# chenxy99/Scanpaths

Hardware: AMD Instinct MI355X
Metric: images/sec/GPU (AiR train step, bs=32, 320x512) at 1/2/4/8 MI355X (higher is better)
Workload: dtype f32; 1 GPU; AiR supervised train step (fwd+loss+bwd+clip+Adam), resnet50, T=16, 320x512, per-GPU batch 32; global_batch=32, parallelism=dp1

## Files before the change

### include/scanpaths_amd.h

```cpp
#ifndef SCANPATHS_AMD_H
#define SCANPATHS_AMD_H
#include <stdint.h>

#ifdef __cplusplus
extern "C" {
#endif

#define SP_OK 0
#define SP_EINVAL (-1)
#define SP_ENULL (-2)

#define SP_ABI_VERSION 4
int sp_abi_version(void);

int sp_set_tuning(const char* name, int value);
int sp_timing_build(void);

typedef struct sp_conv_desc {
    int N_img, Hi, Wi, Kc, ldx;
    int Ho, Wo, Nout, ldc;
    int KH, KW, stride, pad, dil;
    int mode, ldw;
    float alpha;
    int beta, relu;
// ... 125 lines not shown
int sp_sempool_fwd(const float* a, const float* vf, int S, int B, int P, int C, float alpha, void* workspace, float* out, int sbc,
                   void* stream);
int sp_sempool_bwd(const float* dout, const float* out, const float* a, const float* vf, int S, int B, int P, int C, float alpha,
                   float* da, float* dvf, const int* row_last, int row_step, int sbc, void* stream);
int sp_lstm_pointwise_bwd(const float* dh, const float* dc, const float* gates, const float* c_prev, const float* c_out,
                          int64_t rows, int C, float* dpre, float* dc_prev, unsigned* dpre_amax, unsigned* dcp_amax,
                          const unsigned* dh_amax, const unsigned* dc_amax, float c_bound, float cprev_bound, void* planes,
                          float* dpre_scale, const int* row_last, int row_step, int rows_per_sample, void* stream);

int sp_im2col3x3_1ch(const float* maps, int S, int R, int H, int W, int ldk, float* col, void* stream);
int sp_col2im3x3_1ch(const float* dcol, int S, int R, int H, int W, int ldk, float* dmaps, void* stream);

int sp_listatt_fwd(const float* L, const float* u, int T, int R, int D, float* mem, float* alpha, void* stream);
int sp_listatt_bwd(const float* dmem, const float* L, const float* u, const float* alpha, int T, int R, int D, float* dL,
                   float* du_partial, void* stream);

int sp_mulrelu_fwd(const float* a, const float* b, int64_t n, int64_t nb, float* out, void* stream);
int sp_mulrelu_bwd(const float* dout, const float* a, const float* b, const float* out, int64_t n, int64_t nb, float* da,
                   float* db_partial, void* stream);

int sp_select_rows(const float* a, const float* b, const unsigned char* sel, int64_t rows, int64_t len, float* out,
                   void* stream);
int sp_select_rows_bwd(const float* dout, const unsigned char* sel, int64_t rows, int64_t len, float* da, float* db,
                       void* stream);

int sp_head_finish_fwd(const float* Z, int B, int Hm, int Wm, int ldz, int nheads, int HC, const float* cb,
                       int cb_per_sample , const float* w2, const float* b2, int softmax, float* logits, float* amap, float* mu,
                       float* sigma2, float* drt,
                       const float* dpre ,
                       int zc , int parts, void* stream);
int sp_head_finish_bwd(const float* dlogits, int64_t dlogits_ld, const float* damap , const float* dmu,
                       const float* dsigma2, const float* logits, const float* amap, const float* sigma2, const float* drt, int B, int Hm,
                       int Wm, int ldz, int nheads, int HC, const float* w2, int softmax, float* dZ, float* dcb_partial,
                       float* dw2_partial, float* db2_partial,
                       float* ddpre ,
                       int zc, int parts, int* live, void* stream);

int sp_head_num_classes(int Hm, int Wm);
int sp_head_compose11_fwd(const float* G, const float* cb, int nheads, int HC, int C, int Hm, int Wm, float* W11,
                          float* cbsum, void* stream);
int sp_head_compose11_bwd(const float* dW11, const float* dcbsum, int nheads, int HC, int C, int Hm, int Wm, float* dG,
                          float* dcb, void* stream);
int sp_sal_gather_fwd(const float* T, int B, int Hm, int Wm, int ldt, int nsel, const int* hmap, float* Z2, void* stream);
int sp_sal_gather_bwd(const float* dZ2, int B, int Hm, int Wm, int ldt, int nsel, int nsrc, const int* hmap, float* dT,
                      const int* row_last, int row_step, void* stream);
int sp_drt_direct_fwd(const float* h, const float* W11, const float* cbsum, const int* hmap, int B, int Hm, int Wm, int C,
                      int nsel, float* Dpre, void* stream);
int sp_drt_direct_bwd_data(const float* dDpre, const float* W11, const int* hmap, int B, int Hm, int Wm, int C, int nsel,
                           int accumulate, float* dh, const int* live, const int* row_last, int row_step, int rowB, void* stream);
int64_t sp_drt_direct_bwd_weight_workspace(int B, int Hm, int Wm, int C, int nsel);
int sp_drt_direct_bwd_weight(const float* dDpre, const float* h, const int* hmap, int B, int Hm, int Wm, int C, int nsel, int nheads,
                             void* workspace, float* dW11, float* dcbsum, const int* live, const int* row_last, int row_step, int rowB,
                             void* stream);

int sp_gemm_skinny_applies(int M, int N, int K, int lda, int ldb, int ldc, int layout);
int64_t sp_gemm_skinny_workspace(int M, int N, int K, int layout);
int sp_gemm_skinny(const float* A, const float* B, const float* bias, float* C, int M, int N, int K, int lda, int ldb, int ldc, int layout,
                   float alpha, int relu, void* workspace, void* stream);

int64_t sp_scanpath_loss_workspace(int B, int T);
// ... 106 lines not shown
```

### scanpaths_amd/config.py

```python
from __future__ import annotations

import os
import sys

DEFAULTS = {
    "split_scheme": "f16x2", "use_split": True, "library": "product", "always_reset_amax": False,
    "fused_amax": True, "grad_merge": True, "bn_split": True, "bn_skip_dx": True, "bn_skip_z": True, "lstm_bwd_split": True,
    "rank1_dsp_split": True, "rank1_dwc_split": True, "lstm_skip_dpre": True, "fuse_gate_lstm": True, "lstm_h_planes": True,
    "defer_wgrad": True, "channel_scales": True, "hw2_single": True, "row_sparsity": True, "direct_grad": True, "skinny_gemm": True, "async_dgrad": True,
    "drt_batched": True, "rank1_fused": True,
}
_off = lambda v: v != "0"
_ENV = {
    "SP_SPLIT_SCHEME": ("split_scheme", str), "SP_NO_SPLIT": ("use_split", lambda v: not v), "SP_LIBRARY": ("library", str),
    "SP_ALWAYS_RESET_AMAX": ("always_reset_amax", bool), "SP_NO_AMAX_HINT": ("fused_amax", lambda v: not v),
    "SP_GRAD_MERGE": ("grad_merge", _off), "SP_BN_SPLIT": ("bn_split", _off), "SP_BN_SKIP_DX": ("bn_skip_dx", _off),
    "SP_BN_SKIP_Z": ("bn_skip_z", _off), "SP_LSTM_BWD_SPLIT": ("lstm_bwd_split", _off), "SP_RANK1_DSP_SPLIT": ("rank1_dsp_split", _off),
    "SP_RANK1_DWC_SPLIT": ("rank1_dwc_split", _off), "SP_LSTM_SKIP_DPRE": ("lstm_skip_dpre", _off), "SP_FUSE_LSTM": ("fuse_gate_lstm", _off),
    "SP_LSTM_H_PLANES": ("lstm_h_planes", _off), "SP_DEFER_WGRAD": ("defer_wgrad", _off), "SP_CHANNEL_SCALES": ("channel_scales", _off),
    "SP_HW2_SINGLE": ("hw2_single", _off), "SP_ROW_SPARSITY": ("row_sparsity", _off), "SP_DIRECT_GRAD": ("direct_grad", _off), "SP_SKINNY_GEMM": ("skinny_gemm", _off),
    "SP_ASYNC_DGRAD": ("async_dgrad", _off), "SP_DRT_BATCHED": ("drt_batched", _off), "SP_RANK1_FUSED": ("rank1_fused", _off),
}
TIMING_KNOBS = {"SP_H2_DBG": b"h2_dbg", "SP_HW_DBG": b"hw_dbg", "SP_B3_DBG": b"b3_dbg", "SP_HW_SPLITS": b"hw_splits", "SP_H2_HALO": b"h2_halo",
                "SP_ROW_ORDER": b"row_order", "SP_HW_CAP": b"hw_cap"}

settings = dict(DEFAULTS)
_announced = set()


def env_tuning_allowed() -> bool:
    return os.environ.get("SP_ALLOW_ENV_TUNING") == "1"


def _loud(msg: str) -> None:
    if msg not in _announced:
        _announced.add(msg)
# ... 65 lines not shown
```

### scanpaths_amd/csrc/decoder.hip

```cpp
#include "common.h"
#include <algorithm>

namespace {

inline int ew_blocks(int64_t n) { return (int)std::max<int64_t>(1, std::min<int64_t>(sp_cdiv(n, 256), 2048)); }

__device__ __forceinline__ float sigmoidf_(float x) { return sp_sigmoid(x); }

__global__ __launch_bounds__(256) void lstm_fwd_kernel(const float* xg, const float* hg, const float* c_prev,
                                                       int64_t rows, int C, float* gates, float* c_out, float* h_out) {
    const int C4 = C / 4;
    const int64_t total = rows * C4;
    for (int64_t idx = (int64_t)blockIdx.x * blockDim.x + threadIdx.x; idx < total; idx += (int64_t)gridDim.x * blockDim.x) {
        const int64_t r = idx / C4;
        const int c = (int)(idx - r * C4) * 4;
        const float* px = xg + r * 4 * C + c;
        float4 pi = *reinterpret_cast<const float4*>(px);
        float4 pf = *reinterpret_cast<const float4*>(px + C);
        float4 po = *reinterpret_cast<const float4*>(px + 2 * C);
        float4 pg = *reinterpret_cast<const float4*>(px + 3 * C);
        if (hg) {
            const float* ph = hg + r * 4 * C + c;
            const float4 a = *reinterpret_cast<const float4*>(ph), b = *reinterpret_cast<const float4*>(ph + C);
            const float4 d = *reinterpret_cast<const float4*>(ph + 2 * C), e = *reinterpret_cast<const float4*>(ph + 3 * C);
// ... 371 lines not shown
        const int r = (int)(q % R);
        const int s = (int)(q / R);
        float acc = 0.f;
#pragma unroll
        for (int tap = 0; tap < 9; ++tap) {
            const int y0 = y - (tap / 3 - 1), x0 = x - (tap % 3 - 1);
            if ((unsigned)y0 < (unsigned)H && (unsigned)x0 < (unsigned)W)
                acc += dcol[(((int64_t)r * H + y0) * W + x0) * ldk + 9 * s + tap];
        }
        dmaps[i] = acc;
    }
}

constexpr int MAXT = 40;

__global__ __launch_bounds__(256) void listatt_fwd_kernel(const float* L, const float* u, int T, int R, int D, float* mem,
                                                          float* alpha) {
    __shared__ float sh16[16];
    __shared__ float sc[MAXT];
    const int r = blockIdx.x;
    for (int t0 = 0; t0 < T; t0 += 4) {
        float s[4] = {0.f, 0.f, 0.f, 0.f};
        for (int d = threadIdx.x; d < D; d += 256) {
            const float ud = u[d];
#pragma unroll
            for (int k = 0; k < 4; ++k)
                if (t0 + k < T) s[k] += L[((int64_t)(t0 + k) * R + r) * D + d] * ud;
        }
        block_sum4_256(s, sh16);
        if (threadIdx.x == 0) {
#pragma unroll
            for (int k = 0; k < 4; ++k)
                if (t0 + k < T) sc[t0 + k] = s[k];
        }
    }
    __syncthreads();
    float mx = -INFINITY;
    for (int t = 0; t < T; ++t) mx = fmaxf(mx, sc[t]);
    float den = 0.f;
    for (int t = 0; t < T; ++t) den += expf(sc[t] - mx);
    const float inv = 1.f / den;
    if (threadIdx.x < T) alpha[(int64_t)threadIdx.x * R + r] = expf(sc[threadIdx.x] - mx) * inv;
    for (int d = threadIdx.x; d < D; d += 256) {
        float acc = 0.f;
        for (int t = 0; t < T; ++t) acc += expf(sc[t] - mx) * inv * L[((int64_t)t * R + r) * D + d];
        mem[(int64_t)r * D + d] = acc;
    }
}

__global__ __launch_bounds__(256) void listatt_bwd_kernel(const float* dmem, const float* L, const float* u,
                                                          const float* alpha, int T, int R, int D, float* dL,
                                                          float* du_partial) {
    __shared__ float sh16[16];
    __shared__ float gs[MAXT];
    const int r = blockIdx.x;
    const float* dm = dmem + (int64_t)r * D;
    for (int t0 = 0; t0 < T; t0 += 4) {
        float s[4] = {0.f, 0.f, 0.f, 0.f};
        for (int d = threadIdx.x; d < D; d += 256) {
            const float dmd = dm[d];
#pragma unroll
            for (int k = 0; k < 4; ++k)
                if (t0 + k < T) s[k] += L[((int64_t)(t0 + k) * R + r) * D + d] * dmd;
        }
        block_sum4_256(s, sh16);
        if (threadIdx.x == 0) {
#pragma unroll
            for (int k = 0; k < 4; ++k)
                if (t0 + k < T) gs[t0 + k] = s[k];
        }
    }
    __syncthreads();
    float mean = 0.f;
    for (int t = 0; t < T; ++t) mean += alpha[(int64_t)t * R + r] * gs[t];
    for (int d = threadIdx.x; d < D; d += 256) {
        const float dmd = dm[d], ud = u[d];
        float du = 0.f;
        for (int t = 0; t < T; ++t) {
            const float a = alpha[(int64_t)t * R + r];
            const float ds = a * (gs[t] - mean);
            const int64_t o = ((int64_t)t * R + r) * D + d;
            du += ds * L[o];
            dL[o] = a * dmd + ds * ud;
        }
        du_partial[(int64_t)r * D + d] = du;
    }
}

__global__ __launch_bounds__(256) void mulrelu_fwd_kernel(const float* a, const float* b, int64_t n, int64_t nb, float* out) {
    for (int64_t i = (int64_t)blockIdx.x * blockDim.x + threadIdx.x; i < n; i += (int64_t)gridDim.x * blockDim.x)
        out[i] = fmaxf(a[i] * b[i % nb], 0.f);
}
__global__ __launch_bounds__(256) void mulrelu_bwd_kernel(const float* dout, const float* a, const float* b, const float* out,
                                                          int64_t n, int64_t nb, float* da, float* db_partial) {
    for (int64_t i = (int64_t)blockIdx.x * blockDim.x + threadIdx.x; i < n; i += (int64_t)gridDim.x * blockDim.x) {
        const float g = out[i] > 0.f ? dout[i] : 0.f;
        da[i] = g * b[i % nb];
// ... 77 lines not shown
    if (threadIdx.x == 0) {
        mu[hd * B + b] = t0 + b2[0];
        sigma2[hd * B + b] = expf(t1 + b2[1]);
    }
    }
    if (softmax && (parts & 1)) {
        __syncthreads();
        float mx = -INFINITY;
        for (int a = threadIdx.x; a <= P; a += 256) mx = fmaxf(mx, lg[a]);
        mx = block_max_256(mx, sh4);
        float den = 0.f;
        for (int a = threadIdx.x; a <= P; a += 256) den += expf(lg[a] - mx);
        den = block_sum_256(den, sh4);
        const float inv = 1.f / den;
        for (int a = threadIdx.x; a <= P; a += 256) lg[a] = expf(lg[a] - mx) * inv;
    }
}

__device__ __forceinline__ double block_sum_256_d(double v, double* sh4d) {
    v = wave_sum_d(v);
    const int w = threadIdx.x >> 6;
    __syncthreads();
    if ((threadIdx.x & 63) == 0) sh4d[w] = v;
    __syncthreads();
    return sh4d[0] + sh4d[1] + sh4d[2] + sh4d[3];
}

__global__ __launch_bounds__(256) void head_bwd_kernel(const float* dlogits, const float* damap, const float* dmu,
                                                       const float* dsigma2, const float* logits, const float* amap,
                                                       const float* sigma2,
// ... 202 lines not shown
    hipLaunchKernelGGL(im2col1_multi_kernel, dim3(ew_blocks((int64_t)R * H * W * ldk)), dim3(256), 0, (hipStream_t)stream, maps, S, R, H, W, ldk, col);
    SP_LAUNCH_CHECK();
    return SP_OK;
}
extern "C" int sp_col2im3x3_1ch(const float* dcol, int S, int R, int H, int W, int ldk, float* dmaps, void* stream) {
    if (!dcol || !dmaps) return SP_ENULL;
    if (S < 1 || 9 * S > ldk) return SP_EINVAL;
    hipLaunchKernelGGL(col2im1_multi_kernel, dim3(ew_blocks((int64_t)S * R * H * W)), dim3(256), 0, (hipStream_t)stream, dcol, S, R, H, W, ldk, dmaps);
    SP_LAUNCH_CHECK();
    return SP_OK;
}

extern "C" int sp_listatt_fwd(const float* L, const float* u, int T, int R, int D, float* mem, float* alpha, void* stream) {
    if (!L || !u || !mem || !alpha) return SP_ENULL;
    if (T < 1 || T > MAXT) return SP_EINVAL;
    hipLaunchKernelGGL(listatt_fwd_kernel, dim3(R), dim3(256), 0, (hipStream_t)stream, L, u, T, R, D, mem, alpha);
    SP_LAUNCH_CHECK();
    return SP_OK;
}

extern "C" int sp_listatt_bwd(const float* dmem, const float* L, const float* u, const float* alpha, int T, int R, int D,
                              float* dL, float* du_partial, void* stream) {
    if (!dmem || !L || !u || !alpha || !dL || !du_partial) return SP_ENULL;
    if (T < 1 || T > MAXT) return SP_EINVAL;
    hipLaunchKernelGGL(listatt_bwd_kernel, dim3(R), dim3(256), 0, (hipStream_t)stream, dmem, L, u, alpha, T, R, D, dL,
                       du_partial);
    SP_LAUNCH_CHECK();
    return SP_OK;
}

extern "C" int sp_mulrelu_fwd(const float* a, const float* b, int64_t n, int64_t nb, float* out, void* stream) {
    if (!a || !b || !out) return SP_ENULL;
    hipLaunchKernelGGL(mulrelu_fwd_kernel, dim3(ew_blocks(n)), dim3(256), 0, (hipStream_t)stream, a, b, n, nb, out);
    SP_LAUNCH_CHECK();
    return SP_OK;
}

extern "C" int sp_mulrelu_bwd(const float* dout, const float* a, const float* b, const float* out, int64_t n, int64_t nb,
                              float* da, float* db_partial, void* stream) {
    if (!dout || !a || !b || !out || !da || !db_partial) return SP_ENULL;
// ... 50 lines not shown
    if (!dcb_partial) return SP_ENULL;
    if ((parts & 1) && (!dlogits || !logits || !amap || !dZ)) return SP_ENULL;
    if ((parts & 2) && (!dmu || !dsigma2 || !sigma2 || !drt || !w2 || !dw2_partial || !db2_partial)) return SP_ENULL;
    if (parts == 2 && !ddpre) return SP_ENULL;
    const int dh = (Hm + 4 - 7) / 5 + 1, dw = (Wm + 4 - 7) / 5 + 1;
    if (zc <= 0) zc = HC;
    if (HC < 52 || dh * dw > MAXS || dh < 1 || dw < 1 || zc < 2 || ((parts & 2) && !ddpre && zc < 2 + NTAP) || ((parts & 1) && nheads * zc > ldz))
        return SP_EINVAL;
    hipLaunchKernelGGL(head_bwd_kernel, dim3(B, nheads), dim3(256), 0, (hipStream_t)stream, dlogits, damap, dmu, dsigma2, logits,
                       amap,
                       sigma2, drt, B, Hm, Wm, ldz, HC, w2, softmax, dZ, dcb_partial, dw2_partial, db2_partial, dh, dw, ddpre, zc, parts, live,
                       dlogits_ld);
    SP_LAUNCH_CHECK();
    return SP_OK;
}
```

### scanpaths_amd/functional.py

```python
from __future__ import annotations

import ctypes as C
from collections import namedtuple
from typing import Optional

import torch
from torch.autograd import Function

from . import config as _config
from . import hip
from .hip import ConvDesc, WgradDesc, check, ptr


_KSPLIT_MIN_NKT, _KSPLIT_KT = 8, 4


def _timed(key_flops, launch):
    if hip.TIMER is None:
        return launch()
    return hip.TIMER.bracket(*key_flops(), launch)


def _gemm_desc(M, Nout, Kc, *, ldx, ldw, ldc, mode=0, alpha=1.0, beta=0, relu=0, nbatch=1, sX=0, sW=0, sC=0):
    return ConvDesc(N_img=M, Hi=1, Wi=1, Kc=Kc, ldx=ldx, Ho=1, Wo=1, Nout=Nout, ldc=ldc, KH=1, KW=1, stride=1, pad=0, dil=1, mode=mode,
# ... 40 lines not shown
                    2.0 * d.N_img * d.Ho * d.Wo * d.Co * d.KH * d.KW * d.Ci * d.nbatch), launch)


def _apply_config():
    g = globals()
    c = _config.settings
    g["FUSED_AMAX"] = bool(c["fused_amax"])
    g["USE_BF16X3"] = bool(c["use_split"])
    g["THROUGHPUT_MODE"] = c["split_scheme"] == "f16x1"
    g["SPLIT_SCHEME"] = "f16x2" if c["split_scheme"] == "f16x1" else c["split_scheme"]
    for name, key in (("GRAD_MERGE", "grad_merge"), ("BN_SPLIT", "bn_split"), ("BN_SKIP_DX", "bn_skip_dx"), ("BN_SKIP_Z", "bn_skip_z"),
                      ("LSTM_BWD_SPLIT", "lstm_bwd_split"), ("RANK1_DSP_SPLIT", "rank1_dsp_split"), ("RANK1_DWC_SPLIT", "rank1_dwc_split"),
                      ("LSTM_SKIP_DPRE", "lstm_skip_dpre"), ("FUSE_GATE_LSTM", "fuse_gate_lstm"), ("LSTM_H_PLANES", "lstm_h_planes"),
                      ("DEFER_WGRAD", "defer_wgrad"), ("CHANNEL_SCALES", "channel_scales"), ("HW2_SINGLE", "hw2_single"),
                      ("ROW_SPARSITY", "row_sparsity"), ("DIRECT_GRAD", "direct_grad"), ("SKINNY_GEMM", "skinny_gemm"), ("ASYNC_DGRAD", "async_dgrad"),
                      ("DRT_BATCHED", "drt_batched"), ("RANK1_FUSED", "rank1_fused")):
        g[name] = bool(c[key])


_apply_config()


FUSION_COUNTS = {"lstm_bwd_split": 0, "bn_bwd_split_operand": 0, "gateconv_lstm": 0, "gateconv_lstm_hplanes": 0,
                 "bn_fwd_split": 0, "bn_fwd_split_operand": 0, "bn_skip_z": 0, "bn_bwd_split": 0, "bn_skip_dx": 0,
                 "conv_bn_stats": 0, "grad_merge": 0, "rank1_dsp_split": 0, "rank1_dwc_split": 0, "lstm_skip_dpre": 0, "wgrad_multi": 0,
                 "row_sparse_bwd": 0, "fan_in_rows": 0, "direct_grad": 0, "output_gate": 0, "skinny_gemm": 0, "async_dgrad": 0,
                 "drt_fwd_batched": 0, "rank1_fused": 0}


def _grad_slot(param):
    if not DIRECT_GRAD or param is None or not getattr(param, "is_leaf", False) or not param.requires_grad:
        return None
    if getattr(param, "_sp_flat", None) is None:
        return None
    if getattr(param, "_backward_hooks", None):
        return None
    try:
        return param, torch.autograd.graph.get_gradient_edge(param).node
    except Exception:
        return None


# ... 1536 lines not shown
        Lst, u, alpha = ctx.saved_tensors
        dmem = dmem.contiguous()
        T, R, D = Lst.shape
        dL = torch.empty_like(Lst)
        dup = torch.empty((R, D), dtype=torch.float32, device=Lst.device)
        check(hip.lib().sp_listatt_bwd(ptr(dmem), ptr(Lst), ptr(u), ptr(alpha), T, R, D, ptr(dL), ptr(dup), hip.stream()),
              "sp_listatt_bwd")
        du = _colsum_any(dup, D) if ctx.needs_input_grad[1] else None
        return dL, du


def list_attention(Lst, u):
    return _ListAtt.apply(Lst, u)


class _MulRelu(Function):
    @staticmethod
    def forward(ctx, a, b):
        a = a.contiguous()
        b = b.contiguous()
        out = torch.empty_like(a)
        check(hip.lib().sp_mulrelu_fwd(ptr(a), ptr(b), a.numel(), b.numel(), ptr(out), hip.stream()), "sp_mulrelu_fwd")
        ctx.save_for_backward(a, b, out)
        return out

    @staticmethod
    def backward(ctx, dout):
        a, b, out = ctx.saved_tensors
        dout = dout.contiguous()
        da = torch.empty_like(a)
# ... 186 lines not shown
            dlogits = dlogits.contiguous()
        damap = damap.contiguous() if damap is not None else None
        dZ = torch.empty((B, Hm, Wm, ldz), dtype=torch.float32, device=logits.device)
        if ldz != nheads * 2:
            dZ.zero_()
        dcbp = torch.empty((B, nheads * HC), dtype=torch.float32, device=logits.device)
        check(hip.lib().sp_head_finish_bwd(ptr(dlogits), dlogits.stride(1), ptr(damap), None, None, ptr(logits), ptr(amap), None, None,
                                           B, Hm, Wm, ldz, nheads, HC, None, int(softmax), ptr(dZ), ptr(dcbp), None, None, None, 2, 1,
                                           None, hip.stream()), "sp_head_finish_bwd (saliency)")
        dcb = dcbp.view(cbshape) if per_sample else _colsum_any(dcbp, nheads * HC).view(nheads, HC)
        return dZ, dcb, None, None, None, None


def head_sal(Z, cb, nheads, HC, softmax, per_sample=False):
    return _HeadSal.apply(Z, cb, nheads, HC, softmax, per_sample)


def head_num_classes(Hm: int, Wm: int) -> int:
    n = hip.lib().sp_head_num_classes(Hm, Wm)
    if n <= 0:
        raise ValueError(f"unsupported map size {Hm}x{Wm} for the duration branch")
    return n


class _Compose11(Function):
    @staticmethod
    def forward(ctx, G, cb, nheads, HC, hw):
        Gp = _phys(G.detach())
        cb = cb.contiguous()
        C_ = Gp.shape[3]
# ... 244 lines not shown
```

### scanpaths_amd/hip.py

```python
from __future__ import annotations

import ctypes as C
import os
from typing import Optional

import torch

from . import config as _config

_HERE = os.path.dirname(os.path.abspath(__file__))
TIMING_LIB = False
LIB_PATH = ""


def _apply_config():
    global TIMING_LIB, LIB_PATH
    TIMING_LIB = _config.settings["library"] == "timing"
    LIB_PATH = os.path.join(_HERE, "libscanpaths_amd_timing.so" if TIMING_LIB else "libscanpaths_amd.so")


_apply_config()


class ConvDesc(C.Structure):
# ... 72 lines not shown
    "sp_nchw_to_nhwc_pad": (_I, [_P, _I, _I, _I, _I, _I, _P, _P]),
    "sp_pad_lastdim": (_I, [_P, _L, _I, _I, _P, _P]),
    "sp_add": (_I, [_P, _P, _P, _L, _P]),
    "sp_lstm_pointwise_fwd": (_I, [_P, _P, _P, _L, _I, _P, _P, _P, _P]),
    "sp_lstm_rank1_fwd": (_I, [_P, _P, _P, _P, _P, _I, _I, _I, _I, _P, _P, _P, _P, _P]),
    "sp_rank1_dwc_workspace": (_L, [_I, _I, _I, _I]),
    "sp_rank1_dwc": (_I, [_P, _P, _I, _I, _I, _I, _I, _P, _P, _P]),
    "sp_sempool_workspace": (_L, [_I, _I, _I, _I]),
    "sp_sempool_fwd": (_I, [_P, _P, _I, _I, _I, _I, _F, _P, _P, _I, _P]),
    "sp_sempool_bwd": (_I, [_P, _P, _P, _P, _I, _I, _I, _I, _F, _P, _P, _P, _I, _I, _P]),
    "sp_lstm_pointwise_bwd": (_I, [_P, _P, _P, _P, _P, _L, _I, _P, _P, _P, _P, _P, _P, _F, _F, _P, _P, _P, _I, _I, _P]),
    "sp_im2col3x3_1ch": (_I, [_P, _I, _I, _I, _I, _I, _P, _P]),
    "sp_col2im3x3_1ch": (_I, [_P, _I, _I, _I, _I, _I, _P, _P]),
    "sp_listatt_fwd": (_I, [_P, _P, _I, _I, _I, _P, _P, _P]),
    "sp_listatt_bwd": (_I, [_P, _P, _P, _P, _I, _I, _I, _P, _P, _P]),
    "sp_mulrelu_fwd": (_I, [_P, _P, _L, _L, _P, _P]),
    "sp_mulrelu_bwd": (_I, [_P, _P, _P, _P, _L, _L, _P, _P, _P]),
    "sp_select_rows": (_I, [_P, _P, _P, _L, _L, _P, _P]),
    "sp_select_rows_bwd": (_I, [_P, _P, _L, _L, _P, _P, _P]),
    "sp_head_finish_fwd": (_I, [_P, _I, _I, _I, _I, _I, _I, _P, _I, _P, _P, _I, _P, _P, _P, _P, _P, _P, _I, _I, _P]),
    "sp_head_finish_bwd": (_I, [_P, _L, _P, _P, _P, _P, _P, _P, _P, _I, _I, _I, _I, _I, _I, _P, _I, _P, _P, _P, _P, _P, _I,
                                _I, _P, _P]),
    "sp_head_num_classes": (_I, [_I, _I]),
    "sp_head_compose11_fwd": (_I, [_P, _P, _I, _I, _I, _I, _I, _P, _P, _P]),
    "sp_head_compose11_bwd": (_I, [_P, _P, _I, _I, _I, _I, _I, _P, _P, _P]),
    "sp_sal_gather_fwd": (_I, [_P, _I, _I, _I, _I, _I, _P, _P, _P]),
    "sp_sal_gather_bwd": (_I, [_P, _I, _I, _I, _I, _I, _I, _P, _P, _P, _I, _P]),
    "sp_drt_direct_fwd": (_I, [_P, _P, _P, _P, _I, _I, _I, _I, _I, _P, _P]),
    "sp_drt_direct_bwd_data": (_I, [_P, _P, _P, _I, _I, _I, _I, _I, _I, _P, _P, _P, _I, _I, _P]),
    "sp_drt_direct_bwd_weight_workspace": (_L, [_I, _I, _I, _I, _I]),
    "sp_drt_direct_bwd_weight": (_I, [_P, _P, _P, _I, _I, _I, _I, _I, _I, _P, _P, _P, _P, _P, _I, _I, _P]),
    "sp_scanmatch_max_len": (_I, []),
    "sp_scanmatch_submatrix": (_I, [_I, _I, C.c_double, _P, _P, _P]),
    "sp_scanmatch_sequences": (_I, [_P, _I, _P, _P, _I, _I, _I, _I, _I, C.c_double, C.c_double, C.c_double, _P, _I, _P, _P, _P]),
    "sp_scanmatch_score": (_I, [_P, _P, _I, _P, _P, _I, _P, _I, _P, _I, _P, C.c_double, _P, _P]),
    "sp_scanmatch_score_long_workspace": (_L, [_I, _I]),
    "sp_scanmatch_score_long": (_I, [_P, _P, _I, _P, _P, _I, _P, _I, _P, _I, _P, C.c_double, _P, _P, _P]),
    "sp_scanmatch_align": (_I, [_P, _I, _P, _I, _P, _I, _P, C.c_double, _P, _P, _P, _P, _P, _P]),
    "sp_scan_max_fixations": (_I, []),
    "sp_scan_sed_stde": (_I, [_P, _I, _P, _P, _P, _I, _I, _I, _I, C.c_double, _P, _P, _P]),
    "sp_scan_tde": (_I, [_P, _I, _P, _P, _P, _I, _I, _I, C.c_double, _P, _P, _P]),
    "sp_scan_multimatch": (_I, [_P, _I, _P, _P, _P, _I, C.c_double, C.c_double, _P, _P]),
# ... 172 lines not shown
```

### scanpaths_amd/models/scanpath_model.py

```python
from __future__ import annotations

from typing import Dict, List, Optional

import torch
import torch.nn as nn

from .. import functional as F
from ..spec import ARCHS, COCO_OBJECTS, drt_hw, encoder_channels

HC = 64
NTAP = 49


class _Conv(nn.Module):
    def __init__(self, cin, cout, kh, kw=None, bias=True):
        super().__init__()
        kw = kh if kw is None else kw
        self.weight = nn.Parameter(torch.empty(cout, cin, kh, kw).contiguous(memory_format=torch.channels_last))
        if bias:
            self.bias = nn.Parameter(torch.zeros(cout))
        else:
            self.register_parameter("bias", None)


# ... 317 lines not shown
        grad_on = torch.is_grad_enabled()
        sp_defer = F.DeferredGemmWgrad() if (grad_on and self.spatial_embed.weight.requires_grad) else None
        se_defer = F.DeferredGemmWgrad() if (grad_on and self.semantic_embed.weight.requires_grad) else None
        wr_defer = [F.DeferredGemmWgrad() if (grad_on and w.requires_grad) else None for w in Wr]
        spw = [self.spatial_embed.weight] * T if sp_defer is not None else rep(self.spatial_embed.weight, T)
        sew = [self.semantic_embed.weight] * T if se_defer is not None else rep(self.semantic_embed.weight, T)
        spb, seb = rep(self.spatial_embed.bias, T), rep(self.semantic_embed.bias, T)
        mvfs, u_spas, u_sems = rep(mvf, T), rep(u_spa, T), rep(u_sem, T)
        Wrs = [[w] * T if d is not None else rep(w, T) for w, d in zip(Wr, wr_defer)]
        dbatch = F.DrtBatch(T) if F.DRT_BATCHED else None
        Wsals, W11s, cbsums, cbs = rep(Wsal, T), rep(W11, T), rep(cbsum, T), rep(cb, T + (1 if dbatch is not None else 0))
        w2s, b2s = (None, None) if dbatch is not None else (rep(w2, T), rep(b2, T))
        dpres = []
        sal_cache = {}

        def push(amaps, k):
            spf = F.mul_relu(amaps, mvfs.pop())
            sp_list.append(rep(F.linear(spf.view(S * B, P), spw.pop(), spb.pop(), defer=sp_defer), T - k))
            vf4 = vfs.pop()
            pooled = F.semantic_pool(amaps, vf4, step=at(k), sbc=True) if (S <= 2 and Cc <= 512) else \
                F.gemm(amaps.transpose(0, 1).contiguous(), vf4.view(B, P, Cc), None, "kn", alpha=1.0 / P, relu=True).transpose(0, 1).contiguous()
            se_list.append(rep(F.linear(pooled.view(S * B, Cc), sew.pop(), seb.pop(), defer=se_defer), T - k))
            sp_mem = F.list_attention(torch.stack([a.pop() for a in sp_list], 0), u_spas.pop())
            se_mem = F.list_attention(torch.stack([a.pop() for a in se_list], 0), u_sems.pop())
            return sp_mem, se_mem

        a0 = attention_maps.reshape(1, B, P).to(torch.float32)
        sp_mem, se_mem = push(a0.expand(S, B, P).contiguous(), 0)
        h = c = None
        outs = {"logits": [], "amap": [], "mu": [], "s2": []}
        zpad = torch.zeros(B, 3 * 512, KP - 9 * S, device=dev) if KP > 9 * S else None
        wh_cache = {}
        if torch.is_grad_enabled() and Wh.requires_grad:
            wh_cache["defer"] = F.DeferredWgrad()
        Xg_t = F.fanout(Xg, T) if (T > 1 and Xg.requires_grad) else (Xg,) * T
        for t_ in range(T):
            t = at(t_)
            se = se_mem.view(S, B, Cc).unbind(0)
            parts = [F.gemm(se[s], Wrs[s].pop(), None, "nk", defer=wr_defer[s]).view(B, 3 * 512, 9) for s in range(S)]
            wc = torch.cat(parts + ([zpad] if zpad is not None else []), 2)
            spcol = F.im2col3x3(sp_mem.view(S, B, Hm, Wm), KP)
            hslot = (dbatch, t_) if dbatch is not None else None
            if F.gateconv_lstm_fusable(h, Wh, spcol):
                h, c = F.gateconv_lstm(h, Wh, Xg_t[t], c, spcol, wc, wh_cache, step=t, hslot=hslot)
            else:
                hg = F.conv2d(h, Wh, None, pad=1, wcache=wh_cache, step=t) if h is not None else None
                h, c = F.lstm_cell_rank1(Xg_t[t], hg, c, spcol, wc, step=t, hslot=hslot)
            nuse = 3 if t + 1 < T else 2
            h_sal, h_drt, h = (tuple(F.fanout(h, nuse, step=t)) + (None,))[:3] if h.requires_grad else (h, h, h)
            if dbatch is not None:
                Z2 = F.sal_gather(F.conv2d(h_sal, Wsals.pop(), None, pad=0, step=t, wcache=sal_cache), hmap, nh, nsrc, step=t)
                logits, amap = F.head_sal(Z2, cbs.pop(), nh, HC, not self.training, per_sample=per_sample)
                dpres.append(F.drt_direct(h_drt, W11s.pop(), cbsums.pop(), hmap, nh, step=t, batch=dbatch))
            else:
                logits, amap, mu, s2 = self._heads_step(hp, h_sal, h_drt, Wsals.pop(), W11s.pop(), cbsums.pop(), cbs.pop(), w2s.pop(),
                                                        b2s.pop(), step=t)
                outs["mu"].append(mu)
                outs["s2"].append(s2)
            outs["logits"].append(logits)
            outs["amap"].append(amap)
            if t + 1 < T:
                sp_mem, se_mem = push(amap, t + 1)
        stacks = {k: torch.stack(v, 2) for k, v in outs.items() if v}
        if dbatch is not None:
            stacks["mu"], stacks["s2"] = F.drt_heads_batched(dbatch, dpres, cbs.pop(), w2, b2, HC, per_sample=per_sample)
        if rows is not None and any(v.requires_grad for v in stacks.values()):
            keys = list(stacks)
            stacks = dict(zip(keys, F.output_gate(rows, [stacks[k] for k in keys])))
        return stacks

    def forward(self, images, attention_maps=None, third=None):
        if not images.is_cuda:
            raise RuntimeError("scanpaths_amd runs on a HIP device only (no CPU path); move the model and inputs to cuda")
        B = images.shape[0]
        Hm, Wm = self.map_height, self.map_width
        if self.task == "OSIE":
            attention_maps = torch.zeros(B, 1, Hm, Wm, device=images.device)
# ... 22 lines not shown
```

Measured before the change: 142.2 images/s.

## Fuse decoder saliency gather, head and spatial mul-relu; pass list-attention entries by pointer table

Adds a fused saliency-head kernel. It stages the selected conv-output columns in LDS by row band and does the 5x5 gather, bias, ReLU, optional softmax and the spatial mul-relu feature in one launch, replacing the separate gather, head and mul_relu kernels. List attention now takes a table of per-step entry pointers instead of a torch.stack copy, so no stacked tensor is materialised on each decoder step. Both paths sit behind a new default-on config flag. The risks are LDS pressure and occupancy in the banded kernel, and a new backward path that relies on the saved logits and amap.

```diff
diff --git a/include/scanpaths_amd.h b/include/scanpaths_amd.h
--- a/include/scanpaths_amd.h
+++ b/include/scanpaths_amd.h
@@ -163,6 +163,9 @@
 int sp_listatt_fwd(const float* L, const float* u, int T, int R, int D, float* mem, float* alpha, void* stream);
 int sp_listatt_bwd(const float* dmem, const float* L, const float* u, const float* alpha, int T, int R, int D, float* dL,
                    float* du_partial, void* stream);
+int sp_listatt_list_fwd(const float* const* entries, const float* u, int T, int R, int D, float* mem, float* alpha, void* stream);
+int sp_listatt_list_bwd(const float* dmem, const float* const* entries, const float* u, const float* alpha, int T, int R, int D,
+                        float* dL, float* du_partial, void* stream);
 
 int sp_mulrelu_fwd(const float* a, const float* b, int64_t n, int64_t nb, float* out, void* stream);
 int sp_mulrelu_bwd(const float* dout, const float* a, const float* b, const float* out, int64_t n, int64_t nb, float* da,
@@ -193,6 +196,9 @@
 int sp_sal_gather_fwd(const float* T, int B, int Hm, int Wm, int ldt, int nsel, const int* hmap, float* Z2, void* stream);
 int sp_sal_gather_bwd(const float* dZ2, int B, int Hm, int Wm, int ldt, int nsel, int nsrc, const int* hmap, float* dT,
                       const int* row_last, int row_step, void* stream);
+int sp_sal_head_fwd(const float* T, int B, int Hm, int Wm, int ldt, int nsel, int nsrc, const int* hmap, int HC, const float* cb,
+                    int cb_per_sample, const float* mvf , int softmax, float* logits, float* amap,
+                    float* spf , void* stream);
 int sp_drt_direct_fwd(const float* h, const float* W11, const float* cbsum, const int* hmap, int B, int Hm, int Wm, int C,
                       int nsel, float* Dpre, void* stream);
 int sp_drt_direct_bwd_data(const float* dDpre, const float* W11, const int* hmap, int B, int Hm, int Wm, int C, int nsel,
diff --git a/scanpaths_amd/config.py b/scanpaths_amd/config.py
--- a/scanpaths_amd/config.py
+++ b/scanpaths_amd/config.py
@@ -8,7 +8,7 @@
     "fused_amax": True, "grad_merge": True, "bn_split": True, "bn_skip_dx": True, "bn_skip_z": True, "lstm_bwd_split": True,
     "rank1_dsp_split": True, "rank1_dwc_split": True, "lstm_skip_dpre": True, "fuse_gate_lstm": True, "lstm_h_planes": True,
     "defer_wgrad": True, "channel_scales": True, "hw2_single": True, "row_sparsity": True, "direct_grad": True, "skinny_gemm": True, "async_dgrad": True,
-    "drt_batched": True, "rank1_fused": True,
+    "drt_batched": True, "rank1_fused": True, "decode_glue_fused": True,
 }
 _off = lambda v: v != "0"
 _ENV = {
@@ -20,6 +20,7 @@
     "SP_LSTM_H_PLANES": ("lstm_h_planes", _off), "SP_DEFER_WGRAD": ("defer_wgrad", _off), "SP_CHANNEL_SCALES": ("channel_scales", _off),
     "SP_HW2_SINGLE": ("hw2_single", _off), "SP_ROW_SPARSITY": ("row_sparsity", _off), "SP_DIRECT_GRAD": ("direct_grad", _off), "SP_SKINNY_GEMM": ("skinny_gemm", _off),
     "SP_ASYNC_DGRAD": ("async_dgrad", _off), "SP_DRT_BATCHED": ("drt_batched", _off), "SP_RANK1_FUSED": ("rank1_fused", _off),
+    "SP_DECODE_GLUE_FUSED": ("decode_glue_fused", _off),
 }
 TIMING_KNOBS = {"SP_H2_DBG": b"h2_dbg", "SP_HW_DBG": b"hw_dbg", "SP_B3_DBG": b"b3_dbg", "SP_HW_SPLITS": b"hw_splits", "SP_H2_HALO": b"h2_halo",
                 "SP_ROW_ORDER": b"row_order", "SP_HW_CAP": b"hw_cap"}
diff --git a/scanpaths_amd/csrc/decoder.hip b/scanpaths_amd/csrc/decoder.hip
--- a/scanpaths_amd/csrc/decoder.hip
+++ b/scanpaths_amd/csrc/decoder.hip
@@ -409,7 +409,18 @@
 
 constexpr int MAXT = 40;
 
-__global__ __launch_bounds__(256) void listatt_fwd_kernel(const float* L, const float* u, int T, int R, int D, float* mem,
+struct ListStacked {
+    const float* L;
+    int64_t RD;
+    __device__ __forceinline__ const float* at(int t) const { return L + (int64_t)t * RD; }
+};
+struct ListTable {
+    const float* p[MAXT];
+    __device__ __forceinline__ const float* at(int t) const { return p[t]; }
+};
+
+template <class List>
+__global__ __launch_bounds__(256) void listatt_fwd_kernel(List L, const float* u, int T, int R, int D, float* mem,
                                                           float* alpha) {
     __shared__ float sh16[16];
     __shared__ float sc[MAXT];
@@ -420,7 +431,7 @@
             const float ud = u[d];
 #pragma unroll
             for (int k = 0; k < 4; ++k)
-                if (t0 + k < T) s[k] += L[((int64_t)(t0 + k) * R + r) * D + d] * ud;
+                if (t0 + k < T) s[k] += L.at(t0 + k)[(int64_t)r * D + d] * ud;
         }
         block_sum4_256(s, sh16);
         if (threadIdx.x == 0) {
@@ -438,12 +449,13 @@
     if (threadIdx.x < T) alpha[(int64_t)threadIdx.x * R + r] = expf(sc[threadIdx.x] - mx) * inv;
     for (int d = threadIdx.x; d < D; d += 256) {
         float acc = 0.f;
-        for (int t = 0; t < T; ++t) acc += expf(sc[t] - mx) * inv * L[((int64_t)t * R + r) * D + d];
+        for (int t = 0; t < T; ++t) acc += expf(sc[t] - mx) * inv * L.at(t)[(int64_t)r * D + d];
         mem[(int64_t)r * D + d] = acc;
     }
 }
 
-__global__ __launch_bounds__(256) void listatt_bwd_kernel(const float* dmem, const float* L, const float* u,
+template <class List>
+__global__ __launch_bounds__(256) void listatt_bwd_kernel(const float* dmem, List L, const float* u,
                                                           const float* alpha, int T, int R, int D, float* dL,
                                                           float* du_partial) {
     __shared__ float sh16[16];
@@ -456,7 +468,7 @@
             const float dmd = dm[d];
 #pragma unroll
             for (int k = 0; k < 4; ++k)
-                if (t0 + k < T) s[k] += L[((int64_t)(t0 + k) * R + r) * D + d] * dmd;
+                if (t0 + k < T) s[k] += L.at(t0 + k)[(int64_t)r * D + d] * dmd;
         }
         block_sum4_256(s, sh16);
         if (threadIdx.x == 0) {
@@ -475,7 +487,7 @@
             const float a = alpha[(int64_t)t * R + r];
             const float ds = a * (gs[t] - mean);
             const int64_t o = ((int64_t)t * R + r) * D + d;
-            du += ds * L[o];
+            du += ds * L.at(t)[(int64_t)r * D + d];
             dL[o] = a * dmd + ds * ud;
         }
         du_partial[(int64_t)r * D + d] = du;
@@ -583,6 +595,80 @@
         den = block_sum_256(den, sh4);
         const float inv = 1.f / den;
         for (int a = threadIdx.x; a <= P; a += 256) lg[a] = expf(lg[a] - mx) * inv;
+    }
+}
+
+constexpr int SH_COLS = 50, SH_LD = 51;
+
+__global__ __launch_bounds__(256) void sal_head_fwd_kernel(const float* __restrict__ T, int B, int Hm, int Wm, int ldt, int nsel, int nsrc,
+                                                           const int* __restrict__ hmap, int HC, const float* __restrict__ cb,
+                                                           int cb_per_sample, const float* __restrict__ mvf, int softmax, int band,
+                                                           float* logits, float* amap, float* __restrict__ spf) {
+    extern __shared__ float sh_tile[];
+    __shared__ float sh4[4];
+    const int hd = blockIdx.y, b = blockIdx.x, tid = threadIdx.x;
+    const int P = Hm * Wm;
+    const int src = min(max(hmap[b * nsel + hd], 0), nsrc - 1);
+    const int col0 = src * SH_COLS;
+    const int ca = col0 & ~3;
+    const int nv4 = ((col0 + SH_COLS + 3) >> 2) - (ca >> 2);
+    const float* t = T + (int64_t)b * P * ldt + ca;
+    const float* c = cb + (cb_per_sample ? ((int64_t)b * gridDim.y + hd) : (int64_t)hd) * HC;
+    float* lg = logits + ((int64_t)hd * B + b) * (P + 1);
+    float* am = amap + ((int64_t)hd * B + b) * P;
+    float* sp = spf ? spf + ((int64_t)hd * B + b) * P : nullptr;
+    const float* mv = mvf ? mvf + (int64_t)b * P : nullptr;
+    float s0 = 0.f;
+    for (int y0 = 0; y0 < Hm; y0 += band) {
+        const int ya = max(y0 - 2, 0), yb = min(y0 + band + 2, Hm);
+        const int q0 = ya * Wm, nld = (yb - ya) * Wm * nv4;
+        __syncthreads();
+        for (int i = tid; i < nld; i += 256) {
+            const int q = i / nv4, k = i - q * nv4;
+            const float4 v = *reinterpret_cast<const float4*>(t + (int64_t)(q0 + q) * ldt + 4 * k);
+            const float e[4] = {v.x, v.y, v.z, v.w};
+            const int cc = ca + 4 * k - col0;
+#pragma unroll
+            for (int j = 0; j < 4; ++j)
+                if ((unsigned)(cc + j) < (unsigned)SH_COLS) sh_tile[q * SH_LD + cc + j] = e[j];
+        }
+        __syncthreads();
+        const int p0 = y0 * Wm, p1 = min(y0 + band, Hm) * Wm;
+        for (int p = p0 + ((tid - p0) & 255); p < p1; p += 256) {
+            const int py = p / Wm, px = p - py * Wm;
+            float a0 = 0.f, a1 = 0.f;
+            for (int uy = 0; uy < 5; ++uy) {
+                const int qy = py + uy - 2;
+                if ((unsigned)qy >= (unsigned)Hm) continue;
+                for (int ux = 0; ux < 5; ++ux) {
+                    const int qx = px + ux - 2;
+                    if ((unsigned)qx < (unsigned)Wm) {
+                        const float* r = sh_tile + ((qy - ya) * Wm + qx) * SH_LD + uy * 5 + ux;
+                        a0 += r[0];
+                        a1 += r[25];
+                    }
+                }
+            }
+            s0 += a0;
+            const float v = fmaxf(a1 + c[1], 0.f);
+            lg[1 + p] = v;
+            am[p] = v;
+            if (sp) sp[p] = fmaxf(v * mv[p], 0.f);
+        }
+    }
+    s0 = block_sum_256(s0, sh4);
+    const float yterm = s0 / (float)P + c[0];
+    if (tid == 0) lg[0] = yterm;
+    if (softmax) {
+        __syncthreads();
+        float mx = -INFINITY;
+        for (int a = tid; a <= P; a += 256) mx = fmaxf(mx, lg[a]);
+        mx = block_max_256(mx, sh4);
+        float den = 0.f;
+        for (int a = tid; a <= P; a += 256) den += expf(lg[a] - mx);
+        den = block_sum_256(den, sh4);
+        const float inv = 1.f / den;
+        for (int a = tid; a <= P; a += 256) lg[a] = expf(lg[a] - mx) * inv;
     }
 }
 
@@ -815,7 +901,29 @@
 extern "C" int sp_listatt_fwd(const float* L, const float* u, int T, int R, int D, float* mem, float* alpha, void* stream) {
     if (!L || !u || !mem || !alpha) return SP_ENULL;
     if (T < 1 || T > MAXT) return SP_EINVAL;
-    hipLaunchKernelGGL(listatt_fwd_kernel, dim3(R), dim3(256), 0, (hipStream_t)stream, L, u, T, R, D, mem, alpha);
+    hipLaunchKernelGGL(listatt_fwd_kernel<ListStacked>, dim3(R), dim3(256), 0, (hipStream_t)stream, ListStacked{L, (int64_t)R * D}, u, T, R,
+                       D, mem, alpha);
+    SP_LAUNCH_CHECK();
+    return SP_OK;
+}
+
+static int listatt_table(const float* const* entries, int T, ListTable& tab) {
+    if (!entries) return SP_ENULL;
+    if (T < 1 || T > MAXT) return SP_EINVAL;
+    for (int t = 0; t < MAXT; ++t) {
+        tab.p[t] = t < T ? entries[t] : nullptr;
+        if (t < T && !tab.p[t]) return SP_ENULL;
+    }
+    return SP_OK;
+}
+
+extern "C" int sp_listatt_list_fwd(const float* const* entries, const float* u, int T, int R, int D, float* mem, float* alpha,
+                                   void* stream) {
+    if (!u || !mem || !alpha) return SP_ENULL;
+    ListTable tab;
+    const int rc = listatt_table(entries, T, tab);
+    if (rc != SP_OK) return rc;
+    hipLaunchKernelGGL(listatt_fwd_kernel<ListTable>, dim3(R), dim3(256), 0, (hipStream_t)stream, tab, u, T, R, D, mem, alpha);
     SP_LAUNCH_CHECK();
     return SP_OK;
 }
@@ -824,7 +932,19 @@
                               float* dL, float* du_partial, void* stream) {
     if (!dmem || !L || !u || !alpha || !dL || !du_partial) return SP_ENULL;
     if (T < 1 || T > MAXT) return SP_EINVAL;
-    hipLaunchKernelGGL(listatt_bwd_kernel, dim3(R), dim3(256), 0, (hipStream_t)stream, dmem, L, u, alpha, T, R, D, dL,
+    hipLaunchKernelGGL(listatt_bwd_kernel<ListStacked>, dim3(R), dim3(256), 0, (hipStream_t)stream, dmem, ListStacked{L, (int64_t)R * D}, u,
+                       alpha, T, R, D, dL, du_partial);
+    SP_LAUNCH_CHECK();
+    return SP_OK;
+}
+
+extern "C" int sp_listatt_list_bwd(const float* dmem, const float* const* entries, const float* u, const float* alpha, int T, int R,
+                                   int D, float* dL, float* du_partial, void* stream) {
+    if (!dmem || !u || !alpha || !dL || !du_partial) return SP_ENULL;
+    ListTable tab;
+    const int rc = listatt_table(entries, T, tab);
+    if (rc != SP_OK) return rc;
+    hipLaunchKernelGGL(listatt_bwd_kernel<ListTable>, dim3(R), dim3(256), 0, (hipStream_t)stream, dmem, tab, u, alpha, T, R, D, dL,
                        du_partial);
     SP_LAUNCH_CHECK();
     return SP_OK;
@@ -905,3 +1025,27 @@
     SP_LAUNCH_CHECK();
     return SP_OK;
 }
+
+extern "C" int sp_sal_head_fwd(const float* T, int B, int Hm, int Wm, int ldt, int nsel, int nsrc, const int* hmap, int HC,
+                               const float* cb, int cb_per_sample, const float* mvf, int softmax, float* logits, float* amap,
+                               float* spf, void* stream) {
+    if (!T || !hmap || !cb || !logits || !amap) return SP_ENULL;
+    if ((mvf == nullptr) != (spf == nullptr)) return SP_ENULL;
+    if (B < 1 || nsel < 1 || nsrc < 1 || Hm < 1 || Wm < 1 || HC < 2 || ldt % 4 || nsrc * SH_COLS > ldt || ((uintptr_t)T & 15))
+        return SP_EINVAL;
+    constexpr int64_t LDS_CAP = 96 * 1024;
+    const int64_t row_b = (int64_t)Wm * SH_LD * sizeof(float);
+    int band = (int)std::min<int64_t>(LDS_CAP / row_b - 4, Hm);
+    if (band < 1) return SP_EINVAL;
+    const int lds = (int)(std::min(band + 4, Hm) * row_b);
+    static bool attr_set = false;
+    if (!attr_set) {
+        (void)hipFuncSetAttribute(reinterpret_cast<const void*>(sal_head_fwd_kernel), hipFuncAttributeMaxDynamicSharedMemorySize,
+                                  (int)LDS_CAP);
+        attr_set = true;
+    }
+    hipLaunchKernelGGL(sal_head_fwd_kernel, dim3(B, nsel), dim3(256), lds, (hipStream_t)stream, T, B, Hm, Wm, ldt, nsel, nsrc, hmap, HC,
+                       cb, cb_per_sample, mvf, softmax, band, logits, amap, spf);
+    SP_LAUNCH_CHECK();
+    return SP_OK;
+}
diff --git a/scanpaths_amd/functional.py b/scanpaths_amd/functional.py
--- a/scanpaths_amd/functional.py
+++ b/scanpaths_amd/functional.py
@@ -78,7 +78,7 @@
                       ("LSTM_SKIP_DPRE", "lstm_skip_dpre"), ("FUSE_GATE_LSTM", "fuse_gate_lstm"), ("LSTM_H_PLANES", "lstm_h_planes"),
                       ("DEFER_WGRAD", "defer_wgrad"), ("CHANNEL_SCALES", "channel_scales"), ("HW2_SINGLE", "hw2_single"),
                       ("ROW_SPARSITY", "row_sparsity"), ("DIRECT_GRAD", "direct_grad"), ("SKINNY_GEMM", "skinny_gemm"), ("ASYNC_DGRAD", "async_dgrad"),
-                      ("DRT_BATCHED", "drt_batched"), ("RANK1_FUSED", "rank1_fused")):
+                      ("DRT_BATCHED", "drt_batched"), ("RANK1_FUSED", "rank1_fused"), ("DECODE_GLUE_FUSED", "decode_glue_fused")):
         g[name] = bool(c[key])
 
 
@@ -89,7 +89,7 @@
                  "bn_fwd_split": 0, "bn_fwd_split_operand": 0, "bn_skip_z": 0, "bn_bwd_split": 0, "bn_skip_dx": 0,
                  "conv_bn_stats": 0, "grad_merge": 0, "rank1_dsp_split": 0, "rank1_dwc_split": 0, "lstm_skip_dpre": 0, "wgrad_multi": 0,
                  "row_sparse_bwd": 0, "fan_in_rows": 0, "direct_grad": 0, "output_gate": 0, "skinny_gemm": 0, "async_dgrad": 0,
-                 "drt_fwd_batched": 0, "rank1_fused": 0}
+                 "drt_fwd_batched": 0, "rank1_fused": 0, "sal_head_fused": 0}
 
 
 def _grad_slot(param):
@@ -1656,6 +1656,41 @@
     return _ListAtt.apply(Lst, u)
 
 
+class _ListAttList(Function):
+    @staticmethod
+    def forward(ctx, u, *entries):
+        T = len(entries)
+        assert 1 <= T <= 32, T
+        entries = [e.contiguous() for e in entries]
+        u = u.contiguous()
+        R, D = entries[0].shape
+        assert all(e.shape == (R, D) and e.dtype == torch.float32 for e in entries)
+        mem = torch.empty((R, D), dtype=torch.float32, device=u.device)
+        alpha = torch.empty((T, R), dtype=torch.float32, device=u.device)
+        tab = (C.c_void_p * T)(*[e.data_ptr() for e in entries])
+        check(hip.lib().sp_listatt_list_fwd(tab, ptr(u), T, R, D, ptr(mem), ptr(alpha), hip.stream()), "sp_listatt_list_fwd")
+        ctx.save_for_backward(u, alpha, *entries)
+        return mem
+
+    @staticmethod
+    def backward(ctx, dmem):
+        u, alpha, *entries = ctx.saved_tensors
+        dmem = dmem.contiguous()
+        T = len(entries)
+        R, D = entries[0].shape
+        dL = torch.empty((T, R, D), dtype=torch.float32, device=u.device)
+        dup = torch.empty((R, D), dtype=torch.float32, device=u.device)
+        tab = (C.c_void_p * T)(*[e.data_ptr() for e in entries])
+        check(hip.lib().sp_listatt_list_bwd(ptr(dmem), tab, ptr(u), ptr(alpha), T, R, D, ptr(dL), ptr(dup), hip.stream()),
+              "sp_listatt_list_bwd")
+        du = _colsum_any(dup, D) if ctx.needs_input_grad[0] else None
+        return (du,) + dL.unbind(0)
+
+
+def list_attention_entries(entries, u):
+    return _ListAttList.apply(u, *entries)
+
+
 class _MulRelu(Function):
     @staticmethod
     def forward(ctx, a, b):
@@ -1872,6 +1907,74 @@
 
 def head_sal(Z, cb, nheads, HC, softmax, per_sample=False):
     return _HeadSal.apply(Z, cb, nheads, HC, softmax, per_sample)
+
+
+class _SalHead(Function):
+    @staticmethod
+    def forward(ctx, T, hmap, cb, mvf, nsel, nsrc, HC, softmax, per_sample, step):
+        T = T.contiguous()
+        cb = cb.contiguous()
+        B, Hm, Wm, ldt = T.shape
+        P = Hm * Wm
+        logits = torch.empty((nsel, B, P + 1), dtype=torch.float32, device=T.device)
+        amap = torch.empty((nsel, B, P), dtype=torch.float32, device=T.device)
+        spf = torch.empty_like(amap) if mvf is not None else None
+        if mvf is not None:
+            mvf = mvf.contiguous()
+            assert mvf.numel() == B * P
+        check(hip.lib().sp_sal_head_fwd(ptr(T), B, Hm, Wm, ldt, nsel, nsrc, ptr(hmap), HC, ptr(cb), int(per_sample), ptr(mvf), int(softmax),
+                                        ptr(logits), ptr(amap), ptr(spf), hip.stream()), "sp_sal_head_fwd")
+        FUSION_COUNTS["sal_head_fused"] += 1
+        ctx.cfg = (B, Hm, Wm, ldt, nsel, nsrc, HC, softmax, per_sample, tuple(cb.shape))
+        ctx.step = step
+        ctx.save_for_backward(logits, amap, hmap)
+        if spf is None:
+            return logits, amap
+        ctx.mark_non_differentiable(spf)
+        return logits, amap, spf
+
+    @staticmethod
+    def backward(ctx, dlogits, damap, *_):
+        B, Hm, Wm, ldt, nsel, nsrc, HC, softmax, per_sample, cbshape = ctx.cfg
+        logits, amap, hmap = ctx.saved_tensors
+        dev = logits.device
+        if dlogits is None:
+            dlogits = torch.zeros_like(logits)
+        if not (dlogits.stride(2) == 1 and dlogits.stride(0) == B * dlogits.stride(1) and dlogits.stride(1) >= dlogits.shape[2]):
+            dlogits = dlogits.contiguous()
+        damap = damap.contiguous() if damap is not None else None
+        dZ2 = torch.empty((B, Hm, Wm, 2 * nsel), dtype=torch.float32, device=dev)
+        dcbp = torch.empty((B, nsel * HC), dtype=torch.float32, device=dev)
+        check(hip.lib().sp_head_finish_bwd(ptr(dlogits), dlogits.stride(1), ptr(damap), None, None, ptr(logits), ptr(amap), None, None,
+                                           B, Hm, Wm, 2 * nsel, nsel, HC, None, int(softmax), ptr(dZ2), ptr(dcbp), None, None, None, 2, 1,
+                                           None, hip.stream()), "sp_head_finish_bwd (saliency)")
+        dcb = dcbp.view(cbshape) if per_sample else _colsum_any(dcbp, nsel * HC).view(nsel, HC)
+        dT = torch.empty((B, Hm, Wm, ldt), dtype=torch.float32, device=dev)
+        rc = rows_ctx(ctx.step, B)
+        check(hip.lib().sp_sal_gather_bwd(ptr(dZ2), B, Hm, Wm, ldt, nsel, nsrc, ptr(hmap), ptr(dT), ptr(rc.last) if rc is not None else None,
+                                          int(ctx.step) if rc is not None else 0, hip.stream()), "sp_sal_gather_bwd")
+        return dT, None, dcb, None, None, None, None, None, None, None
+
+
+def sal_head(T, hmap, cb, mvf, nsel, nsrc, HC, softmax, per_sample=False, step=None):
+    out = _SalHead.apply(T, hmap, cb, mvf.detach() if mvf is not None else None, nsel, nsrc, HC, softmax, per_sample, step)
+    return out if len(out) == 3 else (out[0], out[1], None)
+
+
+class _MulReluFrom(_MulRelu):
+    @staticmethod
+    def forward(ctx, a, b, out):
+        out = out.view_as(a)
+        ctx.save_for_backward(a.contiguous(), b.contiguous(), out)
+        return out
+
+    @staticmethod
+    def backward(ctx, dout):
+        return _MulRelu.backward(ctx, dout) + (None,)
+
+
+def mul_relu_from(a, b, out):
+    return _MulReluFrom.apply(a, b, out)
 
 
 def head_num_classes(Hm: int, Wm: int) -> int:
diff --git a/scanpaths_amd/hip.py b/scanpaths_amd/hip.py
--- a/scanpaths_amd/hip.py
+++ b/scanpaths_amd/hip.py
@@ -110,6 +110,8 @@
     "sp_col2im3x3_1ch": (_I, [_P, _I, _I, _I, _I, _I, _P, _P]),
     "sp_listatt_fwd": (_I, [_P, _P, _I, _I, _I, _P, _P, _P]),
     "sp_listatt_bwd": (_I, [_P, _P, _P, _P, _I, _I, _I, _P, _P, _P]),
+    "sp_listatt_list_fwd": (_I, [_P, _P, _I, _I, _I, _P, _P, _P]),
+    "sp_listatt_list_bwd": (_I, [_P, _P, _P, _P, _I, _I, _I, _P, _P, _P]),
     "sp_mulrelu_fwd": (_I, [_P, _P, _L, _L, _P, _P]),
     "sp_mulrelu_bwd": (_I, [_P, _P, _P, _P, _L, _L, _P, _P, _P]),
     "sp_select_rows": (_I, [_P, _P, _P, _L, _L, _P, _P]),
@@ -122,6 +124,7 @@
     "sp_head_compose11_bwd": (_I, [_P, _P, _I, _I, _I, _I, _I, _P, _P, _P]),
     "sp_sal_gather_fwd": (_I, [_P, _I, _I, _I, _I, _I, _P, _P, _P]),
     "sp_sal_gather_bwd": (_I, [_P, _I, _I, _I, _I, _I, _I, _P, _P, _P, _I, _P]),
+    "sp_sal_head_fwd": (_I, [_P, _I, _I, _I, _I, _I, _I, _P, _I, _P, _I, _P, _I, _P, _P, _P, _P]),
     "sp_drt_direct_fwd": (_I, [_P, _P, _P, _P, _I, _I, _I, _I, _I, _P, _P]),
     "sp_drt_direct_bwd_data": (_I, [_P, _P, _P, _I, _I, _I, _I, _I, _I, _P, _P, _P, _I, _I, _P]),
     "sp_drt_direct_bwd_weight_workspace": (_L, [_I, _I, _I, _I, _I]),
diff --git a/scanpaths_amd/models/scanpath_model.py b/scanpaths_amd/models/scanpath_model.py
--- a/scanpaths_amd/models/scanpath_model.py
+++ b/scanpaths_amd/models/scanpath_model.py
@@ -355,13 +355,17 @@
         dpres = []
         sal_cache = {}
 
-        def push(amaps, k):
-            spf = F.mul_relu(amaps, mvfs.pop())
+        def push(amaps, k, spf=None):
+            spf = F.mul_relu(amaps, mvfs.pop()) if spf is None else F.mul_relu_from(amaps, mvfs.pop(), spf)
             sp_list.append(rep(F.linear(spf.view(S * B, P), spw.pop(), spb.pop(), defer=sp_defer), T - k))
             vf4 = vfs.pop()
             pooled = F.semantic_pool(amaps, vf4, step=at(k), sbc=True) if (S <= 2 and Cc <= 512) else \
                 F.gemm(amaps.transpose(0, 1).contiguous(), vf4.view(B, P, Cc), None, "kn", alpha=1.0 / P, relu=True).transpose(0, 1).contiguous()
             se_list.append(rep(F.linear(pooled.view(S * B, Cc), sew.pop(), seb.pop(), defer=se_defer), T - k))
+            if F.DECODE_GLUE_FUSED:
+                sp_mem = F.list_attention_entries([a.pop() for a in sp_list], u_spas.pop())
+                se_mem = F.list_attention_entries([a.pop() for a in se_list], u_sems.pop())
+                return sp_mem, se_mem
             sp_mem = F.list_attention(torch.stack([a.pop() for a in sp_list], 0), u_spas.pop())
             se_mem = F.list_attention(torch.stack([a.pop() for a in se_list], 0), u_sems.pop())
             return sp_mem, se_mem
@@ -389,9 +393,15 @@
                 h, c = F.lstm_cell_rank1(Xg_t[t], hg, c, spcol, wc, step=t, hslot=hslot)
             nuse = 3 if t + 1 < T else 2
             h_sal, h_drt, h = (tuple(F.fanout(h, nuse, step=t)) + (None,))[:3] if h.requires_grad else (h, h, h)
+            spf = None
             if dbatch is not None:
-                Z2 = F.sal_gather(F.conv2d(h_sal, Wsals.pop(), None, pad=0, step=t, wcache=sal_cache), hmap, nh, nsrc, step=t)
-                logits, amap = F.head_sal(Z2, cbs.pop(), nh, HC, not self.training, per_sample=per_sample)
+                Tp = F.conv2d(h_sal, Wsals.pop(), None, pad=0, step=t, wcache=sal_cache)
+                if F.DECODE_GLUE_FUSED:
+                    logits, amap, spf = F.sal_head(Tp, hmap, cbs.pop(), mvf if t + 1 < T else None, nh, nsrc, HC, not self.training,
+                                                   per_sample=per_sample, step=t)
+                else:
+                    logits, amap = F.head_sal(F.sal_gather(Tp, hmap, nh, nsrc, step=t), cbs.pop(), nh, HC, not self.training,
+                                              per_sample=per_sample)
                 dpres.append(F.drt_direct(h_drt, W11s.pop(), cbsums.pop(), hmap, nh, step=t, batch=dbatch))
             else:
                 logits, amap, mu, s2 = self._heads_step(hp, h_sal, h_drt, Wsals.pop(), W11s.pop(), cbsums.pop(), cbs.pop(), w2s.pop(),
@@ -401,7 +411,7 @@
             outs["logits"].append(logits)
             outs["amap"].append(amap)
             if t + 1 < T:
-                sp_mem, se_mem = push(amap, t + 1)
+                sp_mem, se_mem = push(amap, t + 1, spf)
         stacks = {k: torch.stack(v, 2) for k, v in outs.items() if v}
         if dbatch is not None:
             stacks["mu"], stacks["s2"] = F.drt_heads_batched(dbatch, dpres, cbs.pop(), w2, b2, HC, per_sample=per_sample)
```

Result: no change. 142.1 images/s (-0.0%).
